# reubenvanammers/self_play_reinforcement_learning

Hardware: AMD Instinct MI355X
Metric: self-play positions/sec (Connect4, 200 sims/move) (higher is better)
Workload: dtype fp16

## Files before the change

### self_play_reinforcement_learning_amd/csrc/arena_expand.h

```cpp
template <class G>
__global__ __launch_bounds__(64) void k_expand(View v, const float *probs0, const float *values0,
                                               const float *probs1, const float *values1) {
  constexpr int P = G::APAD;
  const int lane = threadIdx.x & (P - 1);
  const int row = (blockIdx.x * blockDim.x + threadIdx.x) / P;
  if (row >= v.T || !row_live(v, row)) return;
  const bool s1 = row >= v.seg1;
  const float *prow = s1 ? probs1 + (size_t)(row - v.seg1) * G::A : probs0 + (size_t)row * G::A;
  const float vrow = s1 ? values1[row - v.seg1] : values0[row];
  const int tree = v.row_tree[row];
  const size_t nb = nbase<G>(v, tree);
  const size_t bb = (size_t)tree * v.cap;
  const int blk = v.used[tree];
  if (blk >= v.cap) {
    if (lane == 0) set_err(v, SPMCTS_ERR_POOL);
    return;
  }
  const int leaf = v.leaf[tree];
  {
    const size_t ci = nb + (size_t)blk * P + lane;
    nd_n<P>(v, ci) = 0;
    nd_w<P>(v, ci) = 0.0;
    nd_p<P>(v, ci) = lane < G::A ? prow[lane] : 0.f;
    nd_c<P>(v, ci) = -1;
    nd_f<P>(v, ci) = 0;
  }
  const int mover = v.lmover[tree];
  const double val = (double)vrow * (double)mover;
  const int plen = v.plen[tree];
  const size_t pb = (size_t)tree * G::MAXD;
  for (int k = lane; k < plen; k += P) {
    const size_t idx = nb + v.pnode[pb + k];
    nd_n<P>(v, idx) = v.pn[pb + k] + 1;
    nd_w<P>(v, idx) = v.pw[pb + k] + val;
  }
  if (lane == 0) {
    nd_vm<P>(v, bb + blk) = legal_mask<G>(Board{v.lpos[tree], v.lneg[tree]});
    nd_c<P>(v, nb + leaf) = blk;
    nd_n<P>(v, nb + leaf) = v.leaf_n[tree] + 1;
    nd_w<P>(v, nb + leaf) = v.leaf_w[tree] + val;
    v.used[tree] = blk + 1;
    v.need[tree] = 0;
    v.cnt[(size_t)tree * C_NCNT + C_NN] += 1;
    v.cnt[(size_t)tree * C_NCNT + C_HWM] = max(v.cnt[(size_t)tree * C_NCNT + C_HWM], (int64_t)(blk + 1));
  }
}

template <class G>
__device__ __forceinline__ void expand_vl_body(View v, const float *probs0, const float *values0,
                                               const float *probs1, const float *values1) {
  constexpr int P = G::APAD;
  constexpr int GPB = 64 / P;
  constexpr int KMAX = P;
  __shared__ int32_t s_node[GPB][G::MAXD], s_n[GPB][G::MAXD], s_vl[GPB][G::MAXD], s_cs[GPB][G::MAXD];
  __shared__ double s_w[GPB][G::MAXD];
  __shared__ int32_t s_pnode[GPB][KMAX][P];
  __shared__ float s_pr[GPB][KMAX][P];
  __shared__ float s_vr[GPB][KMAX];
  const int lane = threadIdx.x & (P - 1);
  const int grp = threadIdx.x / P;
  const int gbase = (threadIdx.x & 63) & ~(P - 1);
  const int tree = (blockIdx.x * blockDim.x + threadIdx.x) / P;
  if (tree >= v.T) return;
  const PathLds pl{s_node[grp], s_n[grp], s_vl[grp], s_cs[grp], s_w[grp]};
  StoreFence sf;
  const int K = v.K;
  const size_t nb = nbase<G>(v, tree);
  const size_t bb = (size_t)tree * v.cap;
  const int psl = tree * K + (lane < K ? lane : 0);
  const int my_need = lane < K ? (int)v.need[psl] : 0;
  const int my_srow = v.srow[psl], my_leaf = v.leaf[psl], my_plen = v.plen[psl];
  const int my_mover = v.lmover[psl];
  const uint64_t my_pos = v.lpos[psl], my_neg = v.lneg[psl];
  {
    int pn[KMAX];
#pragma unroll
    for (int j = 0; j < KMAX; ++j)
      pn[j] = (j < K && lane < G::MAXD) ? v.pnode[(size_t)(tree * K + j) * G::MAXD + lane] : 0;
#pragma unroll
    for (int j = 0; j < KMAX; ++j) s_pnode[grp][j][lane] = pn[j];
  }
  if (!group_or<P>(my_need)) return;
  const int limit = min(v.budget[tree], v.iters);
  int started = v.tstarted[tree];
  const bool refill = started < limit;
  int used = v.used[tree];
  const bool noise = v.noise_on[tree] != 0;
  const double nz = (noise && lane < G::A) ? v.noise[(size_t)tree * P + lane] : 0.0;
  TreeRng rng;
  TreeRoot R;
  if (refill) {
    rng_load(v, tree, rng);
    R = load_root<G>(v, tree);
  }
  {
    float pr[KMAX], vr[KMAX];
// ... 108 lines not shown
      if (refill && plen > 0) {
        R.n += 1;
        R.vl -= 1;
        R.w += val;
      }
      if (refill && plen > 1) {
        if (lane == s_pnode[grp][j][1] - R.cb * P) {
          R.cn += 1;
          R.cw += val;
          R.cvl -= 1;
        }
      } else if (refill && plen == 1) {
        if (lane == leaf - R.cb * P) {
          R.cc = blk;
          R.cn += 1;
          R.cw += val;
        }
      }
      if (refill && fill_slot_vl<G>(v, tree, j, limit, started, R, rng, terr, pl, noise, nz, sc, sf) == SIM_ERROR)
        break;
    }
  }
  if (lane == 0) {
    sc.flush(v.cnt + (size_t)tree * C_NCNT);
  }
  if (refill && lane == 0) {
    v.tstarted[tree] = started;
    if (terr) set_err(v, SPMCTS_ERR_TAPE);
    rng_store(v, tree, rng);
  }
}

template <class G>
__global__ __launch_bounds__(64) void k_expand_vl(View v, const float *probs0, const float *values0,
                                                  const float *probs1, const float *values1) {
  expand_vl_body<G>(v, probs0, values0, probs1, values1);
}

struct PlayOut {
  int action;
  bool recorded;
  double q;
  uint8_t qf64;
};

__device__ __forceinline__ double kahan_sum(const double *p, int n) {
  double s = p[0], c = 0.0;
  for (int i = 1; i < n; ++i) {
    const double y = p[i] - c;
    const double t = s + y;
    c = (t - s) - y;
    s = t;
  }
  return s;
}

template <class G>
__device__ PlayOut play_move_choice(const View &v, int tree, double temp, float *probs_out) {
  constexpr int P = G::APAD;
  const size_t nb = nbase<G>(v, tree);
  const int root = v.root[tree];
  const int cb = nd_c<P>(v, nb + root);
  PlayOut o{0, false, 0.0, 0};
  int n[G::A];
  for (int j = 0; j < G::A; ++j) n[j] = cb >= 0 ? nd_n<P>(v, nb + (size_t)cb * P + j) : 0;
  double t = temp;
  if (v.evaluate) t = t / 20.0;
// ... 128 lines not shown
```

### self_play_reinforcement_learning_amd/csrc/arena_rows.h

```cpp
template <class G>
__device__ __forceinline__ void leaf_key(const View &v, int t, uint64_t &own, uint64_t &opp) {
  const int mover = v.lmover[t];
  own = mover > 0 ? v.lpos[t] : v.lneg[t];
  opp = mover > 0 ? v.lneg[t] : v.lpos[t];
  if (v.tnet[t / v.K]) own |= 1ull << 63;
}

__device__ __forceinline__ uint32_t leaf_hash(uint64_t a, uint64_t b) {
  uint64_t x = a ^ (b * 0x9E3779B97F4A7C15ull);
  x ^= x >> 33;
  x *= 0xff51afd7ed558ccdull;
  x ^= x >> 33;
  x *= 0xc4ceb9fe1a85ec53ull;
  x ^= x >> 33;
  return (uint32_t)x;
}

template <class G>
__global__ __launch_bounds__(256) void k_dedup_insert(View v) {
  const int t = blockIdx.x * blockDim.x + threadIdx.x;
  if (t >= v.NS || !v.need[t]) return;
  uint64_t own, opp;
  leaf_key<G>(v, t, own, opp);
  const unsigned long long mine = ((unsigned long long)v.dgen << 32) | (uint32_t)t;
  unsigned long long *tab = (unsigned long long *)v.dtab;
  uint32_t h = leaf_hash(own, opp) & (uint32_t)v.dmask;
  for (int probe = 0; probe <= v.dmask; ++probe) {
    unsigned long long w = tab[h];
    while ((uint32_t)(w >> 32) != v.dgen) {
      const unsigned long long old = atomicCAS(tab + h, w, mine);
      if (old == w) {
        v.dent[t] = (int)h;
        return;
      }
      w = old;
    }
    uint64_t so, sp;
    leaf_key<G>(v, (int)(uint32_t)w, so, sp);
    if (so == own && sp == opp) {
      atomicMin(tab + h, mine);
      v.dent[t] = (int)h;
      return;
    }
    h = (h + 1) & (uint32_t)v.dmask;
  }
  set_err(v, SPMCTS_ERR_STATE);
}

constexpr int CACHE_PROBES = 32;
constexpr unsigned long long CACHE_READY = 1ull, CACHE_BUSY = 2ull;

constexpr int CACHE_REC = 8;
static_assert(24 + 4 * (C4::A + 1) <= 8 * CACHE_REC && 24 + 4 * (TTT::A + 1) <= 8 * CACHE_REC, "cache record");

// ... 17 lines not shown
__device__ __forceinline__ int cache_find(const View &v, uint64_t own, uint64_t opp) {
  uint32_t h = leaf_hash(own, opp) & (uint32_t)v.cmask;
  for (int p = 0; p < CACHE_PROBES; ++p) {
    const unsigned long long *r = cache_rec(v, h);
    const unsigned long long tag = r[0];
    if (tag == 0) return -1;
    if (cache_live_tag(v, tag) && r[1] == own && r[2] == opp) {
      __atomic_thread_fence(__ATOMIC_ACQUIRE);
      unsigned long long *rw = cache_rec(v, h);
      const unsigned long long t2 = __hip_atomic_load(rw, __ATOMIC_ACQUIRE, __HIP_MEMORY_SCOPE_AGENT);
      const unsigned long long o2 = __hip_atomic_load(rw + 1, __ATOMIC_RELAXED, __HIP_MEMORY_SCOPE_AGENT);
      const unsigned long long q2 = __hip_atomic_load(rw + 2, __ATOMIC_RELAXED, __HIP_MEMORY_SCOPE_AGENT);
      return cache_live_tag(v, t2) && o2 == own && q2 == opp ? (int)h : -1;
    }
    h = (h + 1) & (uint32_t)v.cmask;
  }
  return -1;
}

template <class G>
__device__ __forceinline__ bool cache_hit(const View &v, int t) {
  uint64_t own, opp;
  leaf_key<G>(v, t, own, opp);
  const int e = cache_find(v, own, opp);
  if (e < 0) return false;
  __hip_atomic_store(cache_rec(v, e), ((unsigned long long)v.cgen << 32) | CACHE_READY, __ATOMIC_RELAXED,
                     __HIP_MEMORY_SCOPE_AGENT);
  v.xc[t] = e;
  return true;
}

template <class G>
__global__ __launch_bounds__(256) void k_dedup_owner(View v) {
  const int t = blockIdx.x * blockDim.x + threadIdx.x;
  if (t >= v.NS) return;
  const bool own = v.need[t] && (int)(uint32_t)v.dtab[v.dent[t]] == t;
  v.down[t] = own ? (v.cwin && cache_hit<G>(v, t) ? 3 : 1) : 0;
  if (own && v.lead) {
    uint64_t a, b;
    leaf_key<G>(v, t, a, b);
    v.okey[2 * (size_t)t] = a;
    v.okey[2 * (size_t)t + 1] = b;
  }
}

template <class G>
__global__ __launch_bounds__(256) void k_dedup_owner_peer(View v, const uint64_t *ptab, const uint64_t *pkey,
                                                          const uint8_t *pdown, int pmask, uint32_t pgen) {
  const int t = blockIdx.x * blockDim.x + threadIdx.x;
  if (t >= v.NS) return;
  int d = 0, xp = -1;
  if (v.need[t] && (int)(uint32_t)v.dtab[v.dent[t]] == t) {
    d = 1;
    if (v.cwin && cache_hit<G>(v, t)) {
      v.down[t] = 3;
      v.xpeer[t] = -1;
      return;
    }
    uint64_t own, opp;
    leaf_key<G>(v, t, own, opp);
    uint32_t h = leaf_hash(own, opp) & (uint32_t)pmask;
    for (int probe = 0; probe <= pmask; ++probe) {
      const unsigned long long w = ptab[h];
      if ((uint32_t)(w >> 32) != pgen) break;
      const int s = (int)(uint32_t)w;
      if (pkey[2 * (size_t)s] == own && pkey[2 * (size_t)s + 1] == opp) {
        if (pdown[s] == 1) {
          d = 2;
          xp = s;
        }
        break;
      }
      h = (h + 1) & (uint32_t)pmask;
    }
  }
  v.down[t] = (uint8_t)d;
  v.xpeer[t] = xp;
}

__global__ __launch_bounds__(256) void k_peer_push(View v, const int32_t *psrow, const float *pprobs,
                                                   const float *pvalues, float *probs, float *values) {
  const int t = blockIdx.x * blockDim.x + threadIdx.x;
  if (t >= v.NS || v.down[t] != 2) return;
  const int r1 = v.srow[t], r0 = psrow[v.xpeer[t]];
  for (int a = 0; a < v.A; ++a) probs[(size_t)r1 * v.A + a] = pprobs[(size_t)r0 * v.A + a];
  values[r1] = pvalues[r0];
}

template <class G>
__global__ __launch_bounds__(256) void k_cache_io(View v, float *probs0, float *values0, float *probs1,
                                                  float *values1) {
  const int t = blockIdx.x * blockDim.x + threadIdx.x;
  if (t >= v.NS || !v.need[t]) return;
  const int d = v.down[t];
  if (d == 0) return;
  const int A = v.A;
  const int row = v.srow[t];
  const bool n1 = row >= v.seg1;
  const int r = n1 ? row - v.seg1 : row;
  float *values = n1 ? values1 : values0;
  float *pr = (n1 ? probs1 : probs0) + (size_t)r * A;
  if (d == 3) {
    const float *c = cache_out(v, v.xc[t]);
    for (int a = 0; a < A; ++a) pr[a] = c[a];
    values[r] = c[A];
    return;
  }
  if (d == 2 && v.cshared) return;
  uint64_t own, opp;
  leaf_key<G>(v, t, own, opp);
  uint32_t h = leaf_hash(own, opp) & (uint32_t)v.cmask;
  const unsigned long long gen = (unsigned long long)v.cgen << 32;
  for (int p = 0; p < CACHE_PROBES; ++p) {
    unsigned long long *rec = cache_rec(v, h);
    unsigned long long w = __hip_atomic_load(rec, __ATOMIC_RELAXED, __HIP_MEMORY_SCOPE_AGENT);
    while (cache_free_tag(v, w)) {
      const unsigned long long old = atomicCAS(rec, w, gen | CACHE_BUSY);
      if (old == w) {
        rec[1] = own;
        rec[2] = opp;
        float *c = cache_out(v, h);
        for (int a = 0; a < A; ++a) c[a] = pr[a];
        c[A] = values[r];
        __hip_atomic_store(rec, gen | CACHE_READY, __ATOMIC_RELEASE, __HIP_MEMORY_SCOPE_AGENT);
        return;
      }
      w = old;
    }
    h = (h + 1) & (uint32_t)v.cmask;
  }
}

__device__ __forceinline__ bool row_owner(const View &v, int t) { return v.dedup ? v.down[t] == 1 : v.need[t] != 0; }

__global__ __launch_bounds__(256) void k_dedup_alias(View v) {
  const int t = blockIdx.x * blockDim.x + threadIdx.x;
  if (t >= v.NS || !v.need[t]) return;
  const int s = (int)(uint32_t)v.dtab[v.dent[t]];
  if (s != t) v.srow[t] = v.srow[s];
}

constexpr int SCAN_THREADS = 512;
constexpr int SCAN_WAVES = SCAN_THREADS / 64;

__global__ __launch_bounds__(SCAN_THREADS) void k_scan_need(View v, int32_t *count_out) {
  __shared__ int32_t s_w0[SCAN_WAVES], s_w1[SCAN_WAVES], s_w2[SCAN_WAVES], s_w4[SCAN_WAVES];
  const int tid = threadIdx.x, lane = tid & 63, wave = tid >> 6;
  const int T = v.NS;
  const int chunk = (T + SCAN_THREADS - 1) / SCAN_THREADS;
  const int lo = min(T, tid * chunk), hi = min(T, lo + chunk);
  int c0 = 0, c1 = 0, c2 = 0, c3 = 0, c4 = 0;
  const bool two = v.seg1 < v.NS;
  if (v.served) {
#pragma unroll 16
    for (int t = lo; t < hi; ++t) {
      const int d = v.down[t];
      const bool n1 = two && v.tnet[t / v.K] != 0;
      c0 += d == 1 && !n1;
      c1 += d == 1 && n1;
      c2 += d >= 2 && !n1;
      c4 += d >= 2 && n1;
      c3 += d == 3;
    }
  } else {
#pragma unroll 16
    for (int t = lo; t < hi; ++t)
      if (row_owner(v, t)) {
        if (v.tnet[t / v.K]) ++c1; else ++c0;
      }
  }
  int i0 = c0, i1 = c1, i2 = c2, i4 = c4;
#pragma unroll
  for (int off = 1; off < 64; off <<= 1) {
    const int a0 = __shfl_up(i0, off, 64), a1 = __shfl_up(i1, off, 64), a2 = __shfl_up(i2, off, 64);
    const int a4 = __shfl_up(i4, off, 64);
    if (lane >= off) {
      i0 += a0;
      i1 += a1;
      i2 += a2;
      i4 += a4;
    }
  }
  if (lane == 63) {
    s_w0[wave] = i0;
    s_w1[wave] = i1;
    s_w2[wave] = i2;
    s_w4[wave] = i4;
  }
  __syncthreads();
  if (wave == 0) {
    int w0 = lane < SCAN_WAVES ? s_w0[lane] : 0, w1 = lane < SCAN_WAVES ? s_w1[lane] : 0;
    int w2 = lane < SCAN_WAVES ? s_w2[lane] : 0, w4 = lane < SCAN_WAVES ? s_w4[lane] : 0;
#pragma unroll
    for (int off = 1; off < SCAN_WAVES; off <<= 1) {
      const int a0 = __shfl_up(w0, off, 64), a1 = __shfl_up(w1, off, 64), a2 = __shfl_up(w2, off, 64);
      const int a4 = __shfl_up(w4, off, 64);
      if (lane >= off) {
        w0 += a0;
        w1 += a1;
        w2 += a2;
        w4 += a4;
      }
    }
    if (lane < SCAN_WAVES) {
      s_w0[lane] = w0;
      s_w1[lane] = w1;
      s_w2[lane] = w2;
      s_w4[lane] = w4;
    }
  }
  __syncthreads();
  i0 += wave ? s_w0[wave - 1] : 0;
  i1 += wave ? s_w1[wave - 1] : 0;
  i2 += wave ? s_w2[wave - 1] : 0;
  i4 += wave ? s_w4[wave - 1] : 0;
  int r0 = i0 - c0, r1 = v.seg1 + i1 - c1;
  if (v.served) {
    int r2 = s_w0[SCAN_WAVES - 1] + i2 - c2, r4 = v.seg1 + s_w1[SCAN_WAVES - 1] + i4 - c4;
#pragma unroll 16
    for (int t = lo; t < hi; ++t) {
      const int d = v.down[t];
      if (d == 0) continue;
      const bool n1 = two && v.tnet[t / v.K] != 0;
      if (d == 1) {
        const int r = n1 ? r1++ : r0++;
        v.row_tree[r] = t;
        v.srow[t] = r;
      } else {
        v.srow[t] = n1 ? r4++ : r2++;
      }
    }
    if (v.cwin) {
#pragma unroll
      for (int off = 32; off > 0; off >>= 1) c3 += __shfl_xor(c3, off, 64);
      if (lane == 0 && c3) atomicAdd((unsigned long long *)&v.gcnt[11], (unsigned long long)c3);
    }
  } else {
#pragma unroll 16
    for (int t = lo; t < hi; ++t)
      if (row_owner(v, t)) {
        const int r = v.tnet[t / v.K] ? r1++ : r0++;
        v.row_tree[r] = t;
        if (v.K > 1) v.srow[t] = r;
      }
  }
  if (tid == SCAN_THREADS - 1) {
    v.row_count[0] = i0;
    v.row_count[1] = i1;
    v.gcnt[10] += i0 + i1;
    if (count_out) {
      count_out[0] = i0 + i1;
      count_out[1] = i0;
      count_out[2] = i1;
    }
  }
}

__device__ __forceinline__ bool row_live(const View &v, int row) {
  return row < v.seg1 ? row < v.row_count[0] : row - v.seg1 < v.row_count[1];
}

template <class G>
__global__ void k_encode(View v, void *out) {
  const int64_t gid = (int64_t)blockIdx.x * blockDim.x + threadIdx.x;
  const int row = (int)(gid / G::CELLS);
  const int cell = (int)(gid % G::CELLS);
  if (row >= v.NS || !row_live(v, row)) return;
  const int t = v.row_tree[row];
  const int x = cell / G::H, y = cell % G::H;
  const uint64_t bit = 1ull << cell_bit<G>(x, y);
  const int mover = v.lmover[t];
  const uint64_t own = mover > 0 ? v.lpos[t] : v.lneg[t];
  const uint64_t opp = mover > 0 ? v.lneg[t] : v.lpos[t];
  const int c_own = (own & bit) ? 1 : 0, c_opp = (opp & bit) ? 1 : 0;
  const int c_emp = 1 - c_own - c_opp;
  if (v.leaf_format == SPMCTS_LEAF_BOARD_I64) {
    ((int64_t *)out)[(size_t)row * G::CELLS + cell] = (int64_t)(c_own - c_opp);
    return;
  }
  size_t i0, i1, i2;
  if (v.leaf_layout == SPMCTS_NHWC) {
    const size_t base = ((size_t)row * G::CELLS + cell) * 3;
    i0 = base;
    i1 = base + 1;
    i2 = base + 2;
  } else {
    const size_t base = (size_t)row * 3 * G::CELLS + cell;
    i0 = base;
    i1 = base + G::CELLS;
    i2 = base + 2 * G::CELLS;
  }
  if (v.leaf_format == SPMCTS_LEAF_F32) {
    float *o = (float *)out;
    o[i0] = (float)c_emp;
    o[i1] = (float)c_own;
    o[i2] = (float)c_opp;
  } else {
    const uint16_t one = v.leaf_format == SPMCTS_LEAF_F16 ? 0x3C00 : 0x3F80;
    uint16_t *o = (uint16_t *)out;
    o[i0] = c_emp ? one : 0;
// ... 5 lines not shown
```

### self_play_reinforcement_learning_amd/csrc/arena_view.h

```cpp
typedef rocrand_state_philox4x32_10 Philox;

struct View {
  int T, cap, G, A;
  int iters;
  int K, NS;
  double cpuct, x, alpha;
  int strong, evaluate, rng_mode, leaf_format, leaf_layout;
  char *nodes;
  int32_t *root;
  uint64_t *rpos, *rneg;
  int8_t *rplayer;
  int32_t *used;
  int32_t gc;
  int32_t *gc_list;
  int32_t *gc_map;
  int32_t *tstarted;
  double *noise;
  uint8_t *noise_on;
  int32_t *pnode;
  int32_t *pn;
  double *pw;
  int32_t *plen;
  int32_t *leaf;
  int32_t *leaf_n;
  double *leaf_w;
  uint64_t *lpos, *lneg;
  int8_t *lmover;
  uint8_t *need;
  Philox *rng;
  const double *tape;
  const int64_t *tape_end;
  int64_t *tape_cur;
  int64_t *cnt;
  int32_t *active;
  int32_t *row_tree;
  int32_t *srow;
  int32_t *row_count;
  uint64_t *dtab;
  int32_t *dent;
  uint8_t *down;
  int dedup, dmask;
  uint32_t dgen;
  uint64_t *okey;
  int32_t *xpeer;
  int lead;
  int peer_on;
  uint64_t *crec;
  int32_t *xc;
  int cwin, cmask;
  uint32_t cgen;
  int cshared;
  int served;
  float *root_prior;
  uint32_t *err;
  uint64_t *gpos, *gneg;
  int32_t *gply;
  uint8_t *gswap, *gstate;
  int8_t *gresult;
  int64_t *gid;
  int8_t *mv_state;
  float *mv_probs;
  double *mv_q;
  uint8_t *mv_qf64;
  int32_t *mv_count;
  int8_t *ex_state;
  float *ex_probs;
  double *ex_q;
  uint8_t *ex_qf64;
  float *ex_z;
  int64_t *ex_game;
  int32_t *ex_count;
  int32_t ex_cap;
  int64_t *gcnt;
  int32_t *gscratch;
  uint8_t *tnet;
  uint8_t *tkind;
  int32_t *budget;
  double *talpha;
  uint8_t *tstrong;
  int32_t *tK;
  int32_t seg1;
  int32_t record;
  int32_t sim;
};

// ... 14 lines not shown
__host__ __device__ __forceinline__ int32_t &nd_vl(const View &v, size_t i) {
  return ((int32_t *)(nd_rec<P>(v, i) + NodeRec<P>::VL))[i % P];
}
template <int P>
__host__ __device__ __forceinline__ int32_t &nd_c(const View &v, size_t i) {
  return ((int32_t *)(nd_rec<P>(v, i) + NodeRec<P>::C))[i % P];
}
template <int P>
__host__ __device__ __forceinline__ float &nd_p(const View &v, size_t i) {
  return ((float *)(nd_rec<P>(v, i) + NodeRec<P>::PR))[i % P];
}
template <int P>
__host__ __device__ __forceinline__ double &nd_w(const View &v, size_t i) {
  return ((double *)(nd_rec<P>(v, i) + NodeRec<P>::W))[i % P];
}
template <int P>
__host__ __device__ __forceinline__ uint8_t &nd_f(const View &v, size_t i) {
  return ((uint8_t *)(nd_rec<P>(v, i) + NodeRec<P>::F))[i % P];
}
template <int P>
__host__ __device__ __forceinline__ uint32_t &nd_vm(const View &v, size_t gb) {
  return *(uint32_t *)(v.nodes + gb * (size_t)NodeRec<P>::BYTES + NodeRec<P>::VM);
}

enum { C_SIMS = 0, C_NN = 1, C_TERM = 2, C_DEPTH = 3, C_SETNODE = 4, C_MOVES = 5, C_LEAK = 6, C_GC = 7, C_HWM = 8, C_NCNT = 10 };
enum { GS_IDLE = 0, GS_ACTIVE = 1, GS_DONE = 2 };

__device__ __forceinline__ void set_err(const View &v, uint32_t f) { atomicOr(v.err, f); }

template <class G>
__device__ __forceinline__ size_t nbase(const View &v, int tree) {
  return (size_t)tree * (size_t)v.cap * G::APAD;
}
```

### self_play_reinforcement_learning_amd/csrc/spmcts.hip

```cpp
#include <hip/hip_runtime.h>
#include <rocrand/rocrand_normal.h>
#include <rocrand/rocrand_philox4x32_10.h>
#include <rocrand/rocrand_uniform.h>

#include "philox.h"

#include <math.h>
#include <stdio.h>
#include <stdlib.h>
#include <string.h>

#include <algorithm>
#include <string>
#include <vector>

#include "board.h"
#include "spmcts.h"

#pragma clang fp contract(off)

using namespace spm;

static thread_local std::string g_last_error;

// ... 9 lines not shown
      return fail(-(int)_e - 1000, std::string(#expr) + ": " + hipGetErrorString(_e));        \
  } while (0)

#define TRY(call)                          \
  do {                                     \
    if (const int _rc = (call)) return _rc; \
  } while (0)

#include "arena_view.h"
#include "arena_rng.h"
#include "arena_select.h"
#include "arena_rows.h"
#include "arena_expand.h"
#include "arena_games.h"
#include "arena_misc.h"

struct spmcts_arena {
  spmcts_config cfg;
  int device;
  int A, W, H, P, cells, maxd, maxm;
  View v;
  std::vector<void *> allocs;
  int n_active;
  spmcts_arena *peer = nullptr;
  std::vector<spmcts_arena *> followers;
  hipEvent_t ev_ins = nullptr, ev_rows = nullptr, ev_push = nullptr, ev_lead = nullptr;
  hipStream_t push_stream = nullptr;
  bool peer_step = false;
  bool push_pending = false;
  std::vector<void *> cache_allocs;
  bool cache_step = false;
  bool cache_shared_step = false;
  const uint64_t *cache_tab = nullptr;
};

static bool cache_view(const spmcts_arena *h, View &v) {
  v.cshared = 0;
  const spmcts_arena *p = h->peer;
  if (!v.cwin || !p || p->v.cwin != v.cwin || !p->v.crec) return false;
  const int d = (int)(v.cgen - p->v.cgen);
  if (d < -1 || d > 1) return false;
  v.crec = p->v.crec;
  v.cmask = p->v.cmask;
  v.cshared = 1;
  return true;
}

template <class F>
static int with_game(int game, int width, int height, const char *unsupported, F &&f) {
  if (game == SPMCTS_CONNECT4 && width == 7 && height == 6) return f(C4{});
  if (game == SPMCTS_TICTACTOE && width == 3 && height == 3) return f(TTT{});
  return fail(-2, unsupported);
}

static int geometry(const spmcts_config *c, int *A, int *P, int *cells, int *maxd, int *maxm) {
  return with_game(c->game, c->width, c->height,
                   "unsupported game/board size (instantiated: connect4 7x6, tictactoe 3x3)", [&](auto g) {
                     using G = decltype(g);
                     *A = G::A; *P = G::APAD; *cells = G::CELLS; *maxd = G::MAXD; *maxm = G::MAXM;
                     return 0;
                   });
}

static int default_cap(const spmcts_config *c, int cells) {
  const long long it = std::max(1, c->iterations);
  const long long cap = 2 + ((cells + 1) / 2) * it + cells + 2;
  return (int)std::min<long long>(cap, 1 << 26);
// ... 22 lines not shown
  View &v = h->v;
  const size_t T = v.T, P = h->P, cap = v.cap, G = v.G;
  pl.add(&v.nodes, T * cap * 32 * P);
  pl.add(&v.root, T);
  pl.add(&v.rpos, T);
  pl.add(&v.rneg, T);
  pl.add(&v.rplayer, T);
  pl.add(&v.used, T);
  pl.add(&v.gc_list, v.gc ? T * cap : 1);
  pl.add(&v.gc_map, v.gc ? T * cap : 1);
  pl.add(&v.tstarted, T);
  pl.add(&v.noise, T * P);
  pl.add(&v.noise_on, T);
  const size_t NS = v.NS;
  pl.add(&v.pnode, NS * h->maxd);
  pl.add(&v.pn, NS * h->maxd);
  pl.add(&v.pw, NS * h->maxd);
  pl.add(&v.plen, NS);
  pl.add(&v.leaf, NS);
  pl.add(&v.leaf_n, NS);
  pl.add(&v.leaf_w, NS);
  pl.add(&v.lpos, NS);
  pl.add(&v.lneg, NS);
  pl.add(&v.lmover, NS);
  pl.add(&v.need, NS);
  pl.add(&v.rng, T);
  pl.add((int64_t **)&v.tape_end, T);
  pl.add(&v.tape_cur, T);
  pl.add(&v.cnt, T * C_NCNT);
  pl.add(&v.active, std::max(T, G));
  pl.add(&v.row_tree, NS);
  pl.add(&v.srow, NS);
  pl.add(&v.row_count, 4);
  {
    size_t tab = 1;
    while (tab < 2 * NS) tab <<= 1;
    v.dmask = (int)(tab - 1);
    pl.add(&v.dtab, v.K > 1 ? tab : 1);
    pl.add(&v.dent, v.K > 1 ? NS : 1);
    pl.add(&v.down, v.K > 1 ? NS : 1);
    pl.add(&v.okey, v.K > 1 ? 2 * NS : 1);
    pl.add(&v.xpeer, v.K > 1 ? NS : 1);
  }
  pl.add(&v.root_prior, 32);
  pl.add(&v.err, 4);
  pl.add(&v.gpos, G);
  pl.add(&v.gneg, G);
  pl.add(&v.gply, G);
  pl.add(&v.gswap, G);
  pl.add(&v.gstate, G);
  pl.add(&v.gresult, G);
  pl.add(&v.gid, G);
  pl.add(&v.mv_state, 2 * G * h->maxm * h->cells);
  pl.add(&v.mv_probs, 2 * G * h->maxm * h->A);
  pl.add(&v.mv_q, 2 * G * h->maxm);
  pl.add(&v.mv_qf64, 2 * G * h->maxm);
  pl.add(&v.mv_count, 2 * G);
  const size_t X = std::max<size_t>(64, 4 * G * h->maxm);
  v.ex_cap = (int32_t)X;
  pl.add(&v.ex_state, X * h->cells);
  pl.add(&v.ex_probs, X * h->A);
  pl.add(&v.ex_q, X);
  pl.add(&v.ex_qf64, X);
  pl.add(&v.ex_z, X);
  pl.add(&v.ex_game, X);
  pl.add(&v.ex_count, 4);
// ... 7 lines not shown
  pl.add(&v.tK, T);
}

static int setup_view(spmcts_arena *h, const spmcts_config *cfg) {
  int A, P, cells, maxd, maxm;
  if (geometry(cfg, &A, &P, &cells, &maxd, &maxm)) return -2;
  h->cfg = *cfg;
  h->A = A;
  h->P = P;
  h->cells = cells;
  h->maxd = maxd;
  h->maxm = maxm;
  h->W = cfg->width;
  h->H = cfg->height;
  View &v = h->v;
  memset(&v, 0, sizeof(v));
  v.T = cfg->n_trees;
  v.G = cfg->n_games;
  v.A = A;
  v.cap = cfg->blocks_per_tree > 0 ? cfg->blocks_per_tree : default_cap(cfg, cells);
  v.gc = v.cap < default_cap(cfg, cells) ? 1 : 0;
  v.cpuct = cfg->cpuct;
  v.x = cfg->x_noise;
  v.alpha = cfg->alpha;
  v.strong = cfg->strong_play;
  v.evaluate = cfg->evaluate;
  v.rng_mode = cfg->rng_mode;
  v.leaf_format = cfg->leaf_format;
  v.leaf_layout = cfg->leaf_layout;
  v.K = std::max(1, cfg->search_threads);
  if (v.K > P) return fail(-3, "search_threads must not exceed the lane group (8 for connect4, 16 for tictactoe)");
  v.iters = std::max(1, cfg->iterations);
  v.NS = v.T * v.K;
  v.seg1 = v.NS;
  v.record = 1;
  v.sim = 0;
  if (v.T <= 0) return fail(-3, "n_trees must be > 0");
  if (v.G < 0 || 2 * (long long)v.G > v.T) return fail(-3, "games mode needs n_trees >= 2 * n_games");
  if (v.T > (1 << 24)) return fail(-3, "too many trees");
  if (v.K > 64 || (long long)v.T * v.K > (1 << 24)) return fail(-3, "search_threads too large");
  if (v.cap < 4) return fail(-3, "blocks_per_tree too small");
  if ((long long)v.cap * P >= (1ll << 31)) return fail(-3, "blocks_per_tree too large");
  return 0;
}

template <class... P, class... A>
static void enqueue(void (*k)(P...), long long n, int B, hipStream_t s, const A &...a) {
  const int blocks = (int)std::max<long long>(1, (n + B - 1) / B);
  hipLaunchKernelGGL(k, dim3(blocks), dim3(B), 0, s, static_cast<P>(a)...);
}
template <class... P, class... A>
static int launch(void (*k)(P...), long long n, int B, hipStream_t s, const A &...a) {
  enqueue(k, n, B, s, a...);
  const hipError_t e = hipGetLastError();
  if (e != hipSuccess) return fail(-(int)e - 1000, std::string("launch: ") + hipGetErrorString(e));
  return 0;
}
#define LAUNCH(h, k, n, B, s, ...) \
  ((h)->cfg.game == SPMCTS_CONNECT4 ? launch(k<C4>, n, B, s, __VA_ARGS__) : launch(k<TTT>, n, B, s, __VA_ARGS__))

extern "C" {

int spmcts_version(void) { return 1; }

const char *spmcts_last_error(void) { return g_last_error.c_str(); }

// ... 71 lines not shown
int spmcts_set_leaf_peer(spmcts_arena *h, spmcts_arena *leader) {
  if (!h) return fail(-1, "null arena");
  if (h->peer) {
    auto &f = h->peer->followers;
    f.erase(std::remove(f.begin(), f.end(), h), f.end());
    h->peer = nullptr;
  }
  h->peer_step = false;
  h->push_pending = false;
  if (!leader) return 0;
  if (leader == h) return fail(-3, "an arena cannot be its own leader");
  if (leader->peer || !h->followers.empty()) return fail(-3, "one level of lanes: a leader cannot follow");
  if (leader->cfg.game != h->cfg.game || leader->device != h->device)
    return fail(-3, "leader and follower must play the same game on the same device");
  if (h->v.K < 2 || leader->v.K != h->v.K) return fail(-3, "cross-lane dedup needs equal search_threads > 1");
  if (h->v.seg1 < h->v.NS || leader->v.seg1 < leader->v.NS) return fail(-3, "cross-lane dedup: single-network arenas");
  for (hipEvent_t *e : {&leader->ev_ins, &h->ev_rows, &h->ev_push, &h->ev_lead})
    if (!*e) HIP_TRY(hipEventCreateWithFlags(e, hipEventDisableTiming));
  leader->followers.push_back(h);
  h->peer = leader;
  return 0;
}

int spmcts_peer_push(spmcts_arena *h, float *probs_dev, float *values_dev, const float *leader_probs_dev,
                     const float *leader_values_dev, spmcts_stream stream, spmcts_stream leader_stream) {
  if (!h) return fail(-1, "null arena");
  if (!h->peer_step) return 0;
  if (!probs_dev || !values_dev || !leader_probs_dev || !leader_values_dev) return fail(-1, "null argument");
  const hipStream_t s = (hipStream_t)stream, ls = (hipStream_t)leader_stream;
  if (!h->push_stream) HIP_TRY(hipStreamCreateWithFlags(&h->push_stream, hipStreamNonBlocking));
  HIP_TRY(hipEventRecord(h->ev_lead, ls));
  HIP_TRY(hipStreamWaitEvent(h->push_stream, h->ev_lead, 0));
  HIP_TRY(hipStreamWaitEvent(h->push_stream, h->ev_rows, 0));
  const int rc = launch(k_peer_push, h->v.NS, 256, h->push_stream, h->v, h->peer->v.srow, leader_probs_dev,
                        leader_values_dev, probs_dev, values_dev);
  HIP_TRY(hipEventRecord(h->ev_push, h->push_stream));
  h->push_pending = true;
  HIP_TRY(hipStreamWaitEvent(s, h->ev_push, 0));
  h->peer_step = false;
  return rc;
}

int spmcts_arena_geometry(const spmcts_arena *h, int32_t *A, int32_t *W, int32_t *H, int32_t *bpt, int32_t *nt,
                          int32_t *ng) {
  if (!h) return fail(-1, "null arena");
  if (A) *A = h->A;
  if (W) *W = h->W;
  if (H) *H = h->H;
  if (bpt) *bpt = h->v.cap;
  if (nt) *nt = h->v.T;
  if (ng) *ng = h->v.G;
  return 0;
}

int spmcts_set_root_prior(spmcts_arena *h, const float *probs_dev, spmcts_stream stream) {
  if (!h || !probs_dev) return fail(-1, "null argument");
  HIP_TRY(hipMemcpyAsync(h->v.root_prior, probs_dev, sizeof(float) * h->A, hipMemcpyDeviceToDevice,
                         (hipStream_t)stream));
  return 0;
}

int spmcts_set_tape(spmcts_arena *h, const double *tape_dev, const int64_t *offsets_dev, spmcts_stream stream) {
  if (!h || !offsets_dev) return fail(-1, "null argument");
  if (h->cfg.rng_mode != SPMCTS_RNG_TAPE) return fail(-4, "arena is not in tape RNG mode");
  h->v.tape = tape_dev;
  return launch(k_set_tape, h->v.T, 256, (hipStream_t)stream, h->v, offsets_dev);
}

int spmcts_tree_reset(spmcts_arena *h, const int32_t *trees_dev, const int8_t *root_player_dev,
                      const float *priors_dev, int32_t n, spmcts_stream stream) {
  if (!h) return fail(-1, "null arena");
  if (n <= 0) return 0;
  return LAUNCH(h, k_tree_reset, n, 128, (hipStream_t)stream, h->v, trees_dev, root_player_dev, priors_dev, n);
}

int spmcts_search_begin(spmcts_arena *h, const int32_t *trees_dev, int32_t n, spmcts_stream stream) {
  if (!h) return fail(-1, "null arena");
  if (n > std::max(h->v.T, h->v.G)) return fail(-3, "too many active trees");
  h->n_active = n;
  h->v.sim = 0;
  if (h->v.cwin) ++h->v.cgen;
  if (n <= 0) return 0;
  TRY(LAUNCH(h, k_search_begin, n, 128, (hipStream_t)stream, h->v, trees_dev, n));
  if (h->v.gc) TRY(LAUNCH(h, k_compact, 256ll * n, 256, (hipStream_t)stream, h->v, n));
  return 0;
}

static bool peer_live(const spmcts_arena *h) { return h->peer && h->v.dedup && h->peer->v.dedup; }

static int launch_rows(spmcts_arena *h, void *leaves_dev, int32_t *leaf_count_dev, hipStream_t s, bool sim_step) {
  h->peer_step = false;
  for (spmcts_arena *f : h->followers)
    if (f->push_pending) {
      HIP_TRY(hipStreamWaitEvent(s, f->ev_push, 0));
      f->push_pending = false;
    }
  View v = h->v;
  v.peer_on = 0;
  h->cache_step = v.cwin > 0 && v.dedup;
  if (!h->cache_step) v.cwin = 0;
  h->cache_shared_step = h->cache_step && cache_view(h, v);
  h->cache_tab = h->cache_step ? v.crec : nullptr;
  v.served = h->cache_step ? 1 : 0;
  if (v.dedup) {
    if (++h->v.dgen == 0) ++h->v.dgen;
    v.dgen = h->v.dgen;
    v.lead = h->followers.empty() ? 0 : 1;
    TRY(LAUNCH(h, k_dedup_insert, v.NS, 256, s, v));
    if (sim_step && peer_live(h)) {
      const spmcts_arena *p = h->peer;
      HIP_TRY(hipStreamWaitEvent(s, p->ev_ins, 0));
      v.peer_on = 1;
      v.served = 1;
      TRY(LAUNCH(h, k_dedup_owner_peer, v.NS, 256, s, v, p->v.dtab, p->v.okey, p->v.down, p->v.dmask, p->v.dgen));
    } else {
      TRY(LAUNCH(h, k_dedup_owner, v.NS, 256, s, v));
    }
    if (v.lead) HIP_TRY(hipEventRecord(h->ev_ins, s));
  }
  TRY(launch(k_scan_need, SCAN_THREADS, SCAN_THREADS, s, v, leaf_count_dev));
  if (v.dedup) TRY(launch(k_dedup_alias, v.NS, 256, s, v));
  if (v.peer_on) {
    HIP_TRY(hipEventRecord(h->ev_rows, s));
    h->peer_step = true;
  }
  if (leaves_dev) TRY(LAUNCH(h, k_encode, (long long)v.NS * h->cells, 256, s, v, leaves_dev));
  return 0;
}

int spmcts_select_tree(spmcts_arena *h, spmcts_stream stream) {
  if (!h) return fail(-1, "null arena");
  hipStream_t s = (hipStream_t)stream;
  const int n = h->n_active;
  int rc = 0;
  if (n > 0) {
    const long long lanes = (long long)n * h->P;
    rc = h->v.K > 1 ? LAUNCH(h, k_select_vl, lanes, 64, s, h->v, n) : LAUNCH(h, k_select, lanes, 64, s, h->v, n);
  }
  h->v.sim += h->v.K;
  return rc;
}

int spmcts_leaf_rows(spmcts_arena *h, void *leaves_dev, int32_t *leaf_count_dev, spmcts_stream stream) {
  if (!h) return fail(-1, "null arena");
  return launch_rows(h, leaves_dev, leaf_count_dev, (hipStream_t)stream, true);
}

int spmcts_select(spmcts_arena *h, void *leaves_dev, int32_t *leaf_count_dev, spmcts_stream stream) {
  const int rc = spmcts_select_tree(h, stream);
  if (rc) return rc;
  return spmcts_leaf_rows(h, leaves_dev, leaf_count_dev, stream);
}

int spmcts_expand2(spmcts_arena *h, const float *probs0_dev, const float *values0_dev, const float *probs1_dev,
                   const float *values1_dev, spmcts_stream stream) {
  if (!h) return fail(-1, "null arena");
  if (h->peer_step) return fail(-4, "a follower lane's simulation step needs spmcts_peer_push before its expand");
  if (h->v.seg1 < h->v.NS && (!probs1_dev || !values1_dev))
    return fail(-1, "two-network arena needs network-1 outputs");
  if (h->cache_step) {
    View v = h->v;
    if (h->cache_shared_step) cache_view(h, v);
    if (v.crec != h->cache_tab) return fail(-4, "the evaluation cache table changed between a step's rows and its expand");
    TRY(LAUNCH(h, k_cache_io, h->v.NS, 256, (hipStream_t)stream, v, (float *)probs0_dev, (float *)values0_dev,
               (float *)probs1_dev, (float *)values1_dev));
    h->cache_step = false;
  }
  const long long lanes = (long long)h->v.T * h->P;
  if (h->v.K > 1)
    return LAUNCH(h, k_expand_vl, lanes, 64, (hipStream_t)stream, h->v, probs0_dev, values0_dev, probs1_dev, values1_dev);
  return LAUNCH(h, k_expand, lanes, 64, (hipStream_t)stream, h->v, probs0_dev, values0_dev, probs1_dev, values1_dev);
}

int spmcts_expand(spmcts_arena *h, const float *probs_dev, const float *values_dev, spmcts_stream stream) {
  if (!h) return fail(-1, "null arena");
  const size_t s1 = (size_t)h->v.seg1;
  const bool dual = h->v.seg1 < h->v.NS;
  return spmcts_expand2(h, probs_dev, values_dev, dual ? probs_dev + s1 * h->A : nullptr,
                        dual ? values_dev + s1 : nullptr, stream);
}

int spmcts_set_tree_players(spmcts_arena *h, const uint8_t *nets, const uint8_t *kinds, const int32_t *budgets) {
  if (!h) return fail(-1, "null arena");
  const int T = h->v.T;
  std::vector<uint8_t> nt(T, 0), kd(T, SPMCTS_PLAYER_MCTS);
  std::vector<int32_t> bd(T, 0x7fffffff);
  int n0 = 0;
  for (int t = 0; t < T; ++t) {
    if (nets) nt[t] = nets[t] ? 1 : 0;
    if (kinds) {
      if (kinds[t] > SPMCTS_PLAYER_LOOKAHEAD) return fail(-3, "unknown player kind");
      kd[t] = kinds[t];
    }
    if (budgets) bd[t] = budgets[t] < 0 ? 0x7fffffff : budgets[t];
    n0 += nt[t] ? 0 : 1;
  }
  HIP_TRY(hipDeviceSynchronize());
  HIP_TRY(hipMemcpy(h->v.tnet, nt.data(), T, hipMemcpyHostToDevice));
  HIP_TRY(hipMemcpy(h->v.tkind, kd.data(), T, hipMemcpyHostToDevice));
  HIP_TRY(hipMemcpy(h->v.budget, bd.data(), 4 * (size_t)T, hipMemcpyHostToDevice));
  h->v.seg1 = n0 * h->v.K;
  return 0;
}
// ... 155 lines not shown
      if (child_p) child_p[j] = 0.f;
    }
  }
  if (board) {
    for (int x = 0; x < h->W; ++x)
      for (int y = 0; y < h->H; ++y) {
        const uint64_t bit = 1ull << (x * (h->H + 1) + y);
        board[x * h->H + y] = (pos & bit) ? 1 : ((neg & bit) ? -1 : 0);
      }
  }
  return 0;
}

int spmcts_games_start(spmcts_arena *h, const int32_t *slots_dev, const float *priors_dev, int32_t n,
                       spmcts_stream stream) {
  if (!h) return fail(-1, "null arena");
  if (h->v.G <= 0) return fail(-4, "arena has no game slots");
  if (n <= 0) return 0;
  hipStream_t s = (hipStream_t)stream;
  TRY(LAUNCH(h, k_games_start, n, 128, s, h->v, slots_dev, priors_dev, n));
  return launch(k_games_bump_id, 1, 1, s, h->v, n);
}

int spmcts_games_set_limit(spmcts_arena *h, int64_t max_games) {
  if (!h) return fail(-1, "null arena");
  HIP_TRY(hipMemcpy(h->v.gcnt + 8, &max_games, 8, hipMemcpyHostToDevice));
  return 0;
}

int spmcts_games_begin_ply(spmcts_arena *h, spmcts_stream stream) {
  if (!h) return fail(-1, "null arena");
  if (h->v.G <= 0) return fail(-4, "arena has no game slots");
  h->n_active = h->v.G;
  h->v.sim = 0;
  if (h->v.cwin) ++h->v.cgen;
  TRY(LAUNCH(h, k_games_begin_ply, h->v.G, 128, (hipStream_t)stream, h->v));
  if (h->v.gc) TRY(LAUNCH(h, k_compact, 256ll * h->v.G, 256, (hipStream_t)stream, h->v, h->v.G));
  return 0;
}

int spmcts_games_end_ply(spmcts_arena *h, void *leaves_dev, int32_t *leaf_count_dev, spmcts_stream stream) {
  if (!h) return fail(-1, "null arena");
  hipStream_t s = (hipStream_t)stream;
  TRY(LAUNCH(h, k_games_end_ply, h->v.G, 64, s, h->v));
  return launch_rows(h, leaves_dev, leaf_count_dev, s, false);
}

int spmcts_games_finish_ply(spmcts_arena *h, int32_t refill, int32_t *out_dev, spmcts_stream stream) {
  if (!h) return fail(-1, "null arena");
  hipStream_t s = (hipStream_t)stream;
  TRY(LAUNCH(h, k_games_finish_scan, 1024, 1024, s, h->v, refill, out_dev));
  return LAUNCH(h, k_games_finish_apply, h->v.G, 64, s, h->v);
}

int spmcts_export_moves(spmcts_arena *h, int8_t *states_dev, float *tree_probs_dev, double *q_dev, uint8_t *q_f64_dev,
                        float *z_dev, int64_t *game_dev, int32_t max_records, int32_t *count_dev,
                        spmcts_stream stream) {
  if (!h) return fail(-1, "null arena");
  hipStream_t s = (hipStream_t)stream;
  TRY(launch(k_export, max_records, 256, s, h->v, h->A, h->cells, states_dev, tree_probs_dev, q_dev, q_f64_dev, z_dev,
             game_dev, max_records, count_dev));
  return launch(k_export_clear, 1, 1, s, h->v);
}

int spmcts_games_state(spmcts_arena *h, uint8_t *active, int32_t *ply, uint8_t *swap, int64_t *game_id) {
  if (!h) return fail(-1, "null arena");
// ... 107 lines not shown
```

Before: 28410.

## Restrict per-step row kernels to the packed active-tree domain

Adds a packed domain (dn, dpack) so the dedup, owner, alias, cache-io, scan, encode and expand kernels iterate only over active trees via an active list instead of all NS slots during game-mode simulation steps. The owner kernel now writes a compact crow array, and the scan reads it in unrolled batches, which also removes the separate served/non-served scan paths. The expand_vl block size grows from 64 to 256 threads. In exchange there is extra indirection through v.active, an owner kernel that now runs even when dedup is off, and more shared memory per expand block.

Measured after the change: 28830 (median of 6 runs). 1.5% higher.

```diff
diff --git a/self_play_reinforcement_learning_amd/csrc/arena_expand.h b/self_play_reinforcement_learning_amd/csrc/arena_expand.h
--- a/self_play_reinforcement_learning_amd/csrc/arena_expand.h
+++ b/self_play_reinforcement_learning_amd/csrc/arena_expand.h
@@ -46,11 +46,13 @@
   }
 }
 
+constexpr int EXPAND_THREADS = 256;
+
 template <class G>
 __device__ __forceinline__ void expand_vl_body(View v, const float *probs0, const float *values0,
                                                const float *probs1, const float *values1) {
   constexpr int P = G::APAD;
-  constexpr int GPB = 64 / P;
+  constexpr int GPB = EXPAND_THREADS / P;
   constexpr int KMAX = P;
   __shared__ int32_t s_node[GPB][G::MAXD], s_n[GPB][G::MAXD], s_vl[GPB][G::MAXD], s_cs[GPB][G::MAXD];
   __shared__ double s_w[GPB][G::MAXD];
@@ -60,8 +62,10 @@
   const int lane = threadIdx.x & (P - 1);
   const int grp = threadIdx.x / P;
   const int gbase = (threadIdx.x & 63) & ~(P - 1);
-  const int tree = (blockIdx.x * blockDim.x + threadIdx.x) / P;
-  if (tree >= v.T) return;
+  const int entry = (blockIdx.x * blockDim.x + threadIdx.x) / P;
+  if (entry >= v.dn) return;
+  const int tree = dom_tree(v, entry);
+  if (tree < 0) return;
   const PathLds pl{s_node[grp], s_n[grp], s_vl[grp], s_cs[grp], s_w[grp]};
   StoreFence sf;
   const int K = v.K;
@@ -236,7 +240,7 @@
 }
 
 template <class G>
-__global__ __launch_bounds__(64) void k_expand_vl(View v, const float *probs0, const float *values0,
+__global__ __launch_bounds__(EXPAND_THREADS) void k_expand_vl(View v, const float *probs0, const float *values0,
                                                   const float *probs1, const float *values1) {
   expand_vl_body<G>(v, probs0, values0, probs1, values1);
 }
diff --git a/self_play_reinforcement_learning_amd/csrc/arena_rows.h b/self_play_reinforcement_learning_amd/csrc/arena_rows.h
--- a/self_play_reinforcement_learning_amd/csrc/arena_rows.h
+++ b/self_play_reinforcement_learning_amd/csrc/arena_rows.h
@@ -18,8 +18,10 @@
 
 template <class G>
 __global__ __launch_bounds__(256) void k_dedup_insert(View v) {
-  const int t = blockIdx.x * blockDim.x + threadIdx.x;
-  if (t >= v.NS || !v.need[t]) return;
+  const int c = blockIdx.x * blockDim.x + threadIdx.x;
+  if (c >= v.dn * v.K) return;
+  const int t = dom_slot(v, c);
+  if (t < 0 || !v.need[t]) return;
   uint64_t own, opp;
   leaf_key<G>(v, t, own, opp);
   const unsigned long long mine = ((unsigned long long)v.dgen << 32) | (uint32_t)t;
@@ -103,29 +105,43 @@
 
 template <class G>
 __global__ __launch_bounds__(256) void k_dedup_owner(View v) {
-  const int t = blockIdx.x * blockDim.x + threadIdx.x;
-  if (t >= v.NS) return;
-  const bool own = v.need[t] && (int)(uint32_t)v.dtab[v.dent[t]] == t;
-  v.down[t] = own ? (v.cwin && cache_hit<G>(v, t) ? 3 : 1) : 0;
-  if (own && v.lead) {
-    uint64_t a, b;
-    leaf_key<G>(v, t, a, b);
-    v.okey[2 * (size_t)t] = a;
-    v.okey[2 * (size_t)t + 1] = b;
-  }
+  const int c = blockIdx.x * blockDim.x + threadIdx.x;
+  if (c >= v.dn * v.K) return;
+  const int t = dom_slot(v, c);
+  int d = 0;
+  if (t >= 0 && !v.dedup) {
+    d = v.need[t] != 0;
+  } else if (t >= 0) {
+    const bool own = v.need[t] && (int)(uint32_t)v.dtab[v.dent[t]] == t;
+    d = own ? (v.cwin && cache_hit<G>(v, t) ? 3 : 1) : 0;
+    v.down[t] = (uint8_t)d;
+    if (own && v.lead) {
+      uint64_t a, b;
+      leaf_key<G>(v, t, a, b);
+      v.okey[2 * (size_t)t] = a;
+      v.okey[2 * (size_t)t + 1] = b;
+    }
+  }
+  v.crow[c] = d ? t * 4 + d : 0;
 }
 
 template <class G>
 __global__ __launch_bounds__(256) void k_dedup_owner_peer(View v, const uint64_t *ptab, const uint64_t *pkey,
                                                           const uint8_t *pdown, int pmask, uint32_t pgen) {
-  const int t = blockIdx.x * blockDim.x + threadIdx.x;
-  if (t >= v.NS) return;
+  const int c = blockIdx.x * blockDim.x + threadIdx.x;
+  if (c >= v.dn * v.K) return;
+  const int t = dom_slot(v, c);
+  if (t < 0) {
+    v.crow[c] = 0;
+    return;
+  }
   int d = 0, xp = -1;
   if (v.need[t] && (int)(uint32_t)v.dtab[v.dent[t]] == t) {
     d = 1;
     if (v.cwin && cache_hit<G>(v, t)) {
       v.down[t] = 3;
       v.xpeer[t] = -1;
+      v.crow[c] = t * 4 + 3;
       return;
     }
     uint64_t own, opp;
@@ -147,12 +163,15 @@
   }
   v.down[t] = (uint8_t)d;
   v.xpeer[t] = xp;
+  v.crow[c] = d ? t * 4 + d : 0;
 }
 
 __global__ __launch_bounds__(256) void k_peer_push(View v, const int32_t *psrow, const float *pprobs,
                                                    const float *pvalues, float *probs, float *values) {
-  const int t = blockIdx.x * blockDim.x + threadIdx.x;
-  if (t >= v.NS || v.down[t] != 2) return;
+  const int c = blockIdx.x * blockDim.x + threadIdx.x;
+  if (c >= v.dn * v.K) return;
+  const int t = dom_slot(v, c);
+  if (t < 0 || v.down[t] != 2) return;
   const int r1 = v.srow[t], r0 = psrow[v.xpeer[t]];
   for (int a = 0; a < v.A; ++a) probs[(size_t)r1 * v.A + a] = pprobs[(size_t)r0 * v.A + a];
   values[r1] = pvalues[r0];
@@ -161,8 +180,10 @@
 template <class G>
 __global__ __launch_bounds__(256) void k_cache_io(View v, float *probs0, float *values0, float *probs1,
                                                   float *values1) {
-  const int t = blockIdx.x * blockDim.x + threadIdx.x;
-  if (t >= v.NS || !v.need[t]) return;
+  const int c = blockIdx.x * blockDim.x + threadIdx.x;
+  if (c >= v.dn * v.K) return;
+  const int t = dom_slot(v, c);
+  if (t < 0 || !v.need[t]) return;
   const int d = v.down[t];
   if (d == 0) return;
   const int A = v.A;
@@ -202,44 +223,53 @@
   }
 }
 
-__device__ __forceinline__ bool row_owner(const View &v, int t) { return v.dedup ? v.down[t] == 1 : v.need[t] != 0; }
-
 __global__ __launch_bounds__(256) void k_dedup_alias(View v) {
-  const int t = blockIdx.x * blockDim.x + threadIdx.x;
-  if (t >= v.NS || !v.need[t]) return;
+  const int c = blockIdx.x * blockDim.x + threadIdx.x;
+  if (c >= v.dn * v.K) return;
+  const int t = dom_slot(v, c);
+  if (t < 0 || !v.need[t]) return;
   const int s = (int)(uint32_t)v.dtab[v.dent[t]];
   if (s != t) v.srow[t] = v.srow[s];
 }
 
 constexpr int SCAN_THREADS = 512;
 constexpr int SCAN_WAVES = SCAN_THREADS / 64;
+constexpr int SCAN_BATCH = 20;
+
+template <class F>
+__device__ __forceinline__ void scan_chunk(const View &v, int lo, int hi, F &&f) {
+  for (int base = lo; base < hi; base += SCAN_BATCH) {
+    int e[SCAN_BATCH];
+    uint32_t n1 = 0;
+#pragma unroll
+    for (int u = 0; u < SCAN_BATCH; ++u) e[u] = v.crow[base + u];
+#pragma unroll
+    for (int u = 0; u < SCAN_BATCH; ++u)
+      if (base + u >= hi) e[u] = 0;
+    if (v.seg1 < v.NS) {
+#pragma unroll
+      for (int u = 0; u < SCAN_BATCH; ++u) n1 |= (v.tnet[(e[u] >> 2) / v.K] ? 1u : 0u) << u;
+    }
+#pragma unroll
+    for (int u = 0; u < SCAN_BATCH; ++u)
+      if (e[u]) f(e[u] >> 2, e[u] & 3, ((n1 >> u) & 1u) != 0);
+  }
+}
 
 __global__ __launch_bounds__(SCAN_THREADS) void k_scan_need(View v, int32_t *count_out) {
   __shared__ int32_t s_w0[SCAN_WAVES], s_w1[SCAN_WAVES], s_w2[SCAN_WAVES], s_w4[SCAN_WAVES];
   const int tid = threadIdx.x, lane = tid & 63, wave = tid >> 6;
-  const int T = v.NS;
+  const int T = v.dn * v.K;
   const int chunk = (T + SCAN_THREADS - 1) / SCAN_THREADS;
   const int lo = min(T, tid * chunk), hi = min(T, lo + chunk);
   int c0 = 0, c1 = 0, c2 = 0, c3 = 0, c4 = 0;
-  const bool two = v.seg1 < v.NS;
-  if (v.served) {
-#pragma unroll 16
-    for (int t = lo; t < hi; ++t) {
-      const int d = v.down[t];
-      const bool n1 = two && v.tnet[t / v.K] != 0;
-      c0 += d == 1 && !n1;
-      c1 += d == 1 && n1;
-      c2 += d >= 2 && !n1;
-      c4 += d >= 2 && n1;
-      c3 += d == 3;
-    }
-  } else {
-#pragma unroll 16
-    for (int t = lo; t < hi; ++t)
-      if (row_owner(v, t)) {
-        if (v.tnet[t / v.K]) ++c1; else ++c0;
-      }
-  }
+  scan_chunk(v, lo, hi, [&](int, int d, bool n1) {
+    c0 += d == 1 && !n1;
+    c1 += d == 1 && n1;
+    c2 += d >= 2 && !n1;
+    c4 += d >= 2 && n1;
+    c3 += d == 3;
+  });
   int i0 = c0, i1 = c1, i2 = c2, i4 = c4;
 #pragma unroll
   for (int off = 1; off < 64; off <<= 1) {
@@ -286,34 +316,20 @@
   i2 += wave ? s_w2[wave - 1] : 0;
   i4 += wave ? s_w4[wave - 1] : 0;
   int r0 = i0 - c0, r1 = v.seg1 + i1 - c1;
-  if (v.served) {
-    int r2 = s_w0[SCAN_WAVES - 1] + i2 - c2, r4 = v.seg1 + s_w1[SCAN_WAVES - 1] + i4 - c4;
-#pragma unroll 16
-    for (int t = lo; t < hi; ++t) {
-      const int d = v.down[t];
-      if (d == 0) continue;
-      const bool n1 = two && v.tnet[t / v.K] != 0;
-      if (d == 1) {
-        const int r = n1 ? r1++ : r0++;
-        v.row_tree[r] = t;
-        v.srow[t] = r;
-      } else {
-        v.srow[t] = n1 ? r4++ : r2++;
-      }
-    }
-    if (v.cwin) {
-#pragma unroll
-      for (int off = 32; off > 0; off >>= 1) c3 += __shfl_xor(c3, off, 64);
-      if (lane == 0 && c3) atomicAdd((unsigned long long *)&v.gcnt[11], (unsigned long long)c3);
-    }
-  } else {
-#pragma unroll 16
-    for (int t = lo; t < hi; ++t)
-      if (row_owner(v, t)) {
-        const int r = v.tnet[t / v.K] ? r1++ : r0++;
-        v.row_tree[r] = t;
-        if (v.K > 1) v.srow[t] = r;
-      }
+  int r2 = s_w0[SCAN_WAVES - 1] + i2 - c2, r4 = v.seg1 + s_w1[SCAN_WAVES - 1] + i4 - c4;
+  scan_chunk(v, lo, hi, [&](int t, int d, bool n1) {
+    if (d == 1) {
+      const int r = n1 ? r1++ : r0++;
+      v.row_tree[r] = t;
+      if (v.K > 1) v.srow[t] = r;
+    } else {
+      v.srow[t] = n1 ? r4++ : r2++;
+    }
+  });
+  if (v.cwin) {
+#pragma unroll
+    for (int off = 32; off > 0; off >>= 1) c3 += __shfl_xor(c3, off, 64);
+    if (lane == 0 && c3) atomicAdd((unsigned long long *)&v.gcnt[11], (unsigned long long)c3);
   }
   if (tid == SCAN_THREADS - 1) {
     v.row_count[0] = i0;
@@ -334,9 +350,10 @@
 template <class G>
 __global__ void k_encode(View v, void *out) {
   const int64_t gid = (int64_t)blockIdx.x * blockDim.x + threadIdx.x;
-  const int row = (int)(gid / G::CELLS);
   const int cell = (int)(gid % G::CELLS);
-  if (row >= v.NS || !row_live(v, row)) return;
+  const int i = (int)(gid / G::CELLS), n0 = v.row_count[0];
+  if (i >= v.dn * v.K || i - n0 >= v.row_count[1]) return;
+  const int row = i < n0 ? i : v.seg1 + i - n0;
   const int t = v.row_tree[row];
   const int x = cell / G::H, y = cell % G::H;
   const uint64_t bit = 1ull << cell_bit<G>(x, y);
diff --git a/self_play_reinforcement_learning_amd/csrc/arena_view.h b/self_play_reinforcement_learning_amd/csrc/arena_view.h
--- a/self_play_reinforcement_learning_amd/csrc/arena_view.h
+++ b/self_play_reinforcement_learning_amd/csrc/arena_view.h
@@ -4,6 +4,7 @@
   int T, cap, G, A;
   int iters;
   int K, NS;
+  int dn, dpack;
   double cpuct, x, alpha;
   int strong, evaluate, rng_mode, leaf_format, leaf_layout;
   char *nodes;
@@ -36,6 +37,7 @@
   int32_t *row_tree;
   int32_t *srow;
   int32_t *row_count;
+  int32_t *crow;
   uint64_t *dtab;
   int32_t *dent;
   uint8_t *down;
@@ -50,7 +52,6 @@
   int cwin, cmask;
   uint32_t cgen;
   int cshared;
-  int served;
   float *root_prior;
   uint32_t *err;
   uint64_t *gpos, *gneg;
@@ -131,3 +132,9 @@
 __device__ __forceinline__ size_t nbase(const View &v, int tree) {
   return (size_t)tree * (size_t)v.cap * G::APAD;
 }
+
+__device__ __forceinline__ int dom_tree(const View &v, int i) { return v.dpack ? v.active[i] : i; }
+__device__ __forceinline__ int dom_slot(const View &v, int c) {
+  const int i = c / v.K, tree = dom_tree(v, i);
+  return tree < 0 ? -1 : tree * v.K + (c - i * v.K);
+}
diff --git a/self_play_reinforcement_learning_amd/csrc/spmcts.hip b/self_play_reinforcement_learning_amd/csrc/spmcts.hip
--- a/self_play_reinforcement_learning_amd/csrc/spmcts.hip
+++ b/self_play_reinforcement_learning_amd/csrc/spmcts.hip
@@ -65,7 +65,14 @@
   bool cache_step = false;
   bool cache_shared_step = false;
   const uint64_t *cache_tab = nullptr;
+  bool games_list = false;
+  bool packed_step = false;
 };
+
+static void set_domain(const spmcts_arena *h, View &v, bool packed) {
+  v.dn = packed ? h->n_active : v.T;
+  v.dpack = packed ? 1 : 0;
+}
 
 static bool cache_view(const spmcts_arena *h, View &v) {
   v.cshared = 0;
@@ -154,6 +161,7 @@
   pl.add(&v.row_tree, NS);
   pl.add(&v.srow, NS);
   pl.add(&v.row_count, 4);
+  pl.add(&v.crow, NS + SCAN_BATCH);
   {
     size_t tab = 1;
     while (tab < 2 * NS) tab <<= 1;
@@ -227,6 +235,8 @@
   if (v.K > P) return fail(-3, "search_threads must not exceed the lane group (8 for connect4, 16 for tictactoe)");
   v.iters = std::max(1, cfg->iterations);
   v.NS = v.T * v.K;
+  v.dn = v.T;
+  v.dpack = 0;
   v.seg1 = v.NS;
   v.record = 1;
   v.sim = 0;
@@ -364,7 +374,9 @@
   HIP_TRY(hipEventRecord(h->ev_lead, ls));
   HIP_TRY(hipStreamWaitEvent(h->push_stream, h->ev_lead, 0));
   HIP_TRY(hipStreamWaitEvent(h->push_stream, h->ev_rows, 0));
-  const int rc = launch(k_peer_push, h->v.NS, 256, h->push_stream, h->v, h->peer->v.srow, leader_probs_dev,
+  View v = h->v;
+  set_domain(h, v, h->packed_step);
+  const int rc = launch(k_peer_push, (long long)v.dn * v.K, 256, h->push_stream, v, h->peer->v.srow, leader_probs_dev,
                         leader_values_dev, probs_dev, values_dev);
   HIP_TRY(hipEventRecord(h->ev_push, h->push_stream));
   h->push_pending = true;
@@ -410,6 +422,7 @@
   if (!h) return fail(-1, "null arena");
   if (n > std::max(h->v.T, h->v.G)) return fail(-3, "too many active trees");
   h->n_active = n;
+  h->games_list = false;
   h->v.sim = 0;
   if (h->v.cwin) ++h->v.cgen;
   if (n <= 0) return 0;
@@ -422,41 +435,44 @@
 
 static int launch_rows(spmcts_arena *h, void *leaves_dev, int32_t *leaf_count_dev, hipStream_t s, bool sim_step) {
   h->peer_step = false;
+  h->packed_step = sim_step && h->games_list;
   for (spmcts_arena *f : h->followers)
     if (f->push_pending) {
       HIP_TRY(hipStreamWaitEvent(s, f->ev_push, 0));
       f->push_pending = false;
     }
   View v = h->v;
+  set_domain(h, v, h->packed_step);
+  const long long slots = (long long)v.dn * v.K;
   v.peer_on = 0;
   h->cache_step = v.cwin > 0 && v.dedup;
   if (!h->cache_step) v.cwin = 0;
   h->cache_shared_step = h->cache_step && cache_view(h, v);
   h->cache_tab = h->cache_step ? v.crec : nullptr;
-  v.served = h->cache_step ? 1 : 0;
   if (v.dedup) {
     if (++h->v.dgen == 0) ++h->v.dgen;
     v.dgen = h->v.dgen;
     v.lead = h->followers.empty() ? 0 : 1;
-    TRY(LAUNCH(h, k_dedup_insert, v.NS, 256, s, v));
+    TRY(LAUNCH(h, k_dedup_insert, slots, 256, s, v));
     if (sim_step && peer_live(h)) {
       const spmcts_arena *p = h->peer;
       HIP_TRY(hipStreamWaitEvent(s, p->ev_ins, 0));
       v.peer_on = 1;
-      v.served = 1;
-      TRY(LAUNCH(h, k_dedup_owner_peer, v.NS, 256, s, v, p->v.dtab, p->v.okey, p->v.down, p->v.dmask, p->v.dgen));
+      TRY(LAUNCH(h, k_dedup_owner_peer, slots, 256, s, v, p->v.dtab, p->v.okey, p->v.down, p->v.dmask, p->v.dgen));
     } else {
-      TRY(LAUNCH(h, k_dedup_owner, v.NS, 256, s, v));
+      TRY(LAUNCH(h, k_dedup_owner, slots, 256, s, v));
     }
     if (v.lead) HIP_TRY(hipEventRecord(h->ev_ins, s));
+  } else {
+    TRY(LAUNCH(h, k_dedup_owner, slots, 256, s, v));
   }
   TRY(launch(k_scan_need, SCAN_THREADS, SCAN_THREADS, s, v, leaf_count_dev));
-  if (v.dedup) TRY(launch(k_dedup_alias, v.NS, 256, s, v));
+  if (v.dedup) TRY(launch(k_dedup_alias, slots, 256, s, v));
   if (v.peer_on) {
     HIP_TRY(hipEventRecord(h->ev_rows, s));
     h->peer_step = true;
   }
-  if (leaves_dev) TRY(LAUNCH(h, k_encode, (long long)v.NS * h->cells, 256, s, v, leaves_dev));
+  if (leaves_dev) TRY(LAUNCH(h, k_encode, slots * h->cells, 256, s, v, leaves_dev));
   return 0;
 }
 
@@ -490,17 +506,20 @@
   if (h->peer_step) return fail(-4, "a follower lane's simulation step needs spmcts_peer_push before its expand");
   if (h->v.seg1 < h->v.NS && (!probs1_dev || !values1_dev))
     return fail(-1, "two-network arena needs network-1 outputs");
+  View dv = h->v;
+  set_domain(h, dv, h->packed_step);
   if (h->cache_step) {
-    View v = h->v;
+    View v = dv;
     if (h->cache_shared_step) cache_view(h, v);
     if (v.crec != h->cache_tab) return fail(-4, "the evaluation cache table changed between a step's rows and its expand");
-    TRY(LAUNCH(h, k_cache_io, h->v.NS, 256, (hipStream_t)stream, v, (float *)probs0_dev, (float *)values0_dev,
-               (float *)probs1_dev, (float *)values1_dev));
+    TRY(LAUNCH(h, k_cache_io, (long long)v.dn * v.K, 256, (hipStream_t)stream, v, (float *)probs0_dev,
+               (float *)values0_dev, (float *)probs1_dev, (float *)values1_dev));
     h->cache_step = false;
   }
+  if (h->v.K > 1)
+    return LAUNCH(h, k_expand_vl, (long long)dv.dn * h->P, EXPAND_THREADS, (hipStream_t)stream, dv, probs0_dev,
+                  values0_dev, probs1_dev, values1_dev);
   const long long lanes = (long long)h->v.T * h->P;
-  if (h->v.K > 1)
-    return LAUNCH(h, k_expand_vl, lanes, 64, (hipStream_t)stream, h->v, probs0_dev, values0_dev, probs1_dev, values1_dev);
   return LAUNCH(h, k_expand, lanes, 64, (hipStream_t)stream, h->v, probs0_dev, values0_dev, probs1_dev, values1_dev);
 }
 
@@ -722,6 +741,7 @@
   if (!h) return fail(-1, "null arena");
   if (h->v.G <= 0) return fail(-4, "arena has no game slots");
   h->n_active = h->v.G;
+  h->games_list = true;
   h->v.sim = 0;
   if (h->v.cwin) ++h->v.cgen;
   TRY(LAUNCH(h, k_games_begin_ply, h->v.G, 128, (hipStream_t)stream, h->v));
```
